# idiap/IdiapTTS

Measured on AMD Instinct MI355X. Metric: acoustic frames/sec (train), higher is better.
Workload: dtype f32

## Files before the change

### idiaptts_amd/csrc/sparse_wgrad.hip

```cpp
#include <algorithm>
#include <atomic>

#include "common.h"

namespace itts {

constexpr int kWgMaxK = 512;
constexpr int kTile = 256;
constexpr int kSlab = 64;
constexpr int kWgWaves = 16;
constexpr int kOwners = 64;
constexpr int kSlots = 8;
constexpr int kStrip = 32;
constexpr int kBlock = 16;
constexpr int kGroup = 4;
constexpr int kHeaderBytes = kSlots * 2;
constexpr int kFirstBytes = kBlock * 8;
constexpr int kOverBytes = (kTile / kBlock - 1) * kBlock * 8;
constexpr int kPlanInv = kStrip + kOwners * kSlots;
constexpr int kPlanInts = kPlanInv + kWgMaxK;
constexpr int kHeavyCode = 0x1000;
constexpr int kRowBytes = kSlab * 4;
constexpr int kBufBytes = (kTile + 1) * kRowBytes;
constexpr int kTPitch = 513;
// ... 40 lines not shown
  if (part == parts) {
    const int h = lane & 31;
    const int hc = h < kStrip - 1 ? plan[h] : -1;
    if (!(hc >= 0 && hc < K)) {
      for (int i = 0; i < 32; ++i) {
        const int64_t m = m0 + 2 * i + (lane >> 5);
        strip[m * kStrip + h] = (m < M && h == kStrip - 1) ? 0x3f800000u : 0u;
      }
    }
    for (int pair = threadIdx.x; pair < kOwners * kSlots; pair += 256) {
      const int c = plan[kStrip + pair];
      if (!(c >= 0 && c < K))
        reinterpret_cast<uint16_t*>(streams + ((int64_t)tile * kOwners + pair / kSlots) * kHeaderBytes)[pair % kSlots] = 0;
    }
    return;
  }
  const int k = part * 64 + lane;
  const bool valid = k < K;
  const int code = valid ? plan[kPlanInv + k] : -1;
  const bool light = code >= 0 && code < kOwners * kSlots;
  const bool heavy = code >= kHeavyCode && code < kHeavyCode + kStrip - 1;
  uint32_t bits[64];
#pragma unroll
  for (int r = 0; r < 64; ++r) bits[r] = (valid && m0 + r < M) ? x[(m0 + r) * ldx + k] : 0u;
  int cnt = 0;
#pragma unroll
  for (int r = 0; r < 64; ++r) cnt += (bits[r] & 0x7fffffffu) != 0u ? 1 : 0;
  cnts[wave][lane] = cnt;
  __syncthreads();
  if (heavy) {
    uint32_t* dst = strip + m0 * kStrip + (code - kHeavyCode);
#pragma unroll
    for (int r = 0; r < 64; ++r) dst[r * kStrip] = bits[r];
  }
  if (!light) return;
  int before = 0, total = 0;
#pragma unroll
  for (int w = 0; w < 4; ++w) {
    const int c = cnts[w][lane];
    before += w < wave ? c : 0;
    total += c;
  }
  const int owner = code / kSlots, slot = code % kSlots;
  const int64_t pair = ((int64_t)tile * kOwners + owner) * kSlots + slot;
  int j = before;
#pragma unroll
  for (int r = 0; r < 64; ++r)
    if ((bits[r] & 0x7fffffffu) != 0u)
      *entry_of(streams, tiles, pair, j++) = make_int2((wave * 64 + r) * kRowBytes, (int)bits[r]);
  if (wave == 0) {
    const int end = (total + kBlock - 1) / kBlock * kBlock;
    for (int e = total; e < end; ++e) *entry_of(streams, tiles, pair, e) = make_int2(kTile * kRowBytes, 0);
    reinterpret_cast<uint16_t*>(streams + ((int64_t)tile * kOwners + owner) * kHeaderBytes)[slot] = (uint16_t)total;
  }
}

typedef float floatx16 __attribute__((ext_vector_type(16)));

template <int J>
__device__ __forceinline__ void col_slot(const char* buf, int lane_off, int2 e, float4& acc) {
  const int off = __builtin_amdgcn_update_dpp(0, e.x, 0x150 + J, 0xf, 0xf, false);
  const float v = __int_as_float(__builtin_amdgcn_update_dpp(0, e.y, 0x150 + J, 0xf, 0xf, false));
  const float4 d = *reinterpret_cast<const float4*>(buf + off + lane_off);
  acc.x = fmaf(v, d.x, acc.x); acc.y = fmaf(v, d.y, acc.y);
  acc.z = fmaf(v, d.z, acc.z); acc.w = fmaf(v, d.w, acc.w);
}
template <int FIRST>
__device__ __forceinline__ void col_group(const char* buf, int lane_off, int2 e, float4& acc) {
  col_slot<FIRST>(buf, lane_off, e, acc);
  col_slot<FIRST + 1>(buf, lane_off, e, acc);
  col_slot<FIRST + 2>(buf, lane_off, e, acc);
  col_slot<FIRST + 3>(buf, lane_off, e, acc);
}

__global__ __launch_bounds__(kWgWaves * 64) void sparse_wgrad_kernel(
    const float* __restrict__ dz, int64_t lddz, const float* __restrict__ strip, const char* __restrict__ streams,
    const int* __restrict__ plan, float* __restrict__ slabs, int64_t slab_stride, int lddw,
    float* __restrict__ bias_part, int64_t bias_stride, int64_t M, int N, int K, int tiles, int per, int ranges) {
  extern __shared__ float4 smem4[];
  char* smem = reinterpret_cast<char*>(smem4);
  float* smemf = reinterpret_cast<float*>(smem4);
  const int tid = threadIdx.x, lane = tid & 63;
  const int wave = __builtin_amdgcn_readfirstlane(tid >> 6);
  const int i16 = lane & 15, owner = wave * 4 + (lane >> 4);
  const int n0 = (int)(blockIdx.x / ranges) * kSlab;
  const int range = (int)(blockIdx.x % ranges);
  const int t_begin = range * per, t_end = std::min(tiles, t_begin + per);

  if (tid < 128) smemf[((tid >> 6) * kBufBytes + kTile * kRowBytes) / 4 + lane] = 0.f;

  const int srow = tid >> 4, c4 = (tid & 15) * 4, n = n0 + c4;
  auto load_tile = [&](int t, float4 (&st)[4]) {
#pragma unroll
    for (int p = 0; p < 4; ++p) {
      const int64_t m = (int64_t)t * kTile + p * 64 + srow;
      float4 v = make_float4(0.f, 0.f, 0.f, 0.f);
      if (m < M) {
        const float* src = dz + m * lddz + n;
        if (n + 4 <= N) {
          v = *reinterpret_cast<const float4*>(src);
        } else {
          if (n < N) v.x = src[0];
          if (n + 1 < N) v.y = src[1];
          if (n + 2 < N) v.z = src[2];
        }
      }
// ... 134 lines not shown
  static int cus = 0;
  if (cus == 0) {
    int dev = 0, n = 0;
    if (hipGetDevice(&dev) != hipSuccess ||
        hipDeviceGetAttribute(&n, hipDeviceAttributeMultiprocessorCount, dev) != hipSuccess || n <= 0)
      n = 256;
    cus = n;
  }
  return cus;
}

static void wgrad_ranges(int64_t M, int N, int* per, int* ranges) {
  const int64_t tiles = (M + kTile - 1) / kTile;
  const int slabs = (N + kSlab - 1) / kSlab;
  const int64_t want = std::max<int64_t>(1, std::min<int64_t>(wgrad_compute_units() / slabs, tiles));
  *per = (int)((tiles + want - 1) / want);
  *ranges = (int)((tiles + *per - 1) / *per);
}

static bool wgrad_shape_ok(int K, int64_t lddw) { return K <= kWgMaxK && lddw <= kWgMaxK; }

}

using namespace itts;

extern "C" int itts_sparse_cols_plan_ints(void) { return kPlanInts; }

extern "C" int itts_sparse_cols_layout(int64_t M, int K, int64_t out[3]) {
  ITTS_REQUIRE(out != nullptr, "null pointer");
  ITTS_REQUIRE(M >= 0 && K > 0 && K <= kWgMaxK, "bad sizes (K <= 512)");
  const ColsLayout l = cols_layout(M);
  out[0] = l.strip_off; out[1] = l.streams_off; out[2] = l.bytes;
  return ITTS_OK;
}

extern "C" int itts_sparse_cols_build(const float* d_x, int64_t ldx, int64_t M, int K, const int* d_plan, void* d_cols,
                                      void* stream) {
  ITTS_REQUIRE(d_plan && d_cols && (M == 0 || d_x), "null pointer");
  ITTS_REQUIRE(M >= 0 && K > 0 && K <= kWgMaxK && ldx >= K, "bad sizes (K <= 512)");
  ITTS_REQUIRE(aligned16(d_cols), "the column block must be 16-byte aligned");
  if (M == 0) return ITTS_OK;
  const ColsLayout l = cols_layout(M);
  const int parts = (K + 63) / 64;
  ITTS_REQUIRE(l.tiles * (parts + 1) < ((int64_t)1 << 31), "too many rows");
  char* base = static_cast<char*>(d_cols);
  hipLaunchKernelGGL(sparse_cols_build_kernel, dim3((unsigned)(l.tiles * (parts + 1))), dim3(256), 0,
                     as_stream(stream), reinterpret_cast<const uint32_t*>(d_x), ldx, M, K, parts, (int)l.tiles, d_plan,
                     reinterpret_cast<uint32_t*>(base + l.strip_off), base + l.streams_off);
  ITTS_LAUNCH_CHECK();
  g_wgrad_path[0].fetch_add(1, std::memory_order_relaxed);
  return ITTS_OK;
}

extern "C" int64_t itts_linear_bwd_weight_sparse_workspace_bytes(int64_t M, int N, int K, int64_t lddw) {
  if (M < 0 || N <= 0 || K <= 0 || lddw < K) return 0;
  const int64_t dense = itts_linear_bwd_weight_workspace_bytes(M, N, (int)lddw);
  if (M == 0 || !wgrad_shape_ok(K, lddw)) return dense;
  int per, ranges;
  wgrad_ranges(M, N, &per, &ranges);
  return std::max<int64_t>(dense, (int64_t)ranges * ((int64_t)N * lddw + N) * 4);
}

extern "C" int itts_linear_bwd_weight_sparse(const float* d_dz, int64_t lddz, const void* d_cols, const int* d_plan,
                                             const float* d_x, int64_t ldx, float* d_dw, int64_t lddw, float* d_db,
                                             int64_t M, int N, int K, void* d_workspace, int accumulate,
                                             void* stream) {
  ITTS_REQUIRE(d_dw && d_workspace && (M == 0 || (d_dz && d_x)), "null pointer");
  ITTS_REQUIRE(M >= 0 && N > 0 && K > 0 && lddz >= N && ldx >= K && lddw >= K, "bad sizes");
  ITTS_REQUIRE(lddw == K || ldx >= lddw, "x must be as wide as dw's rows (its pad columns zero)");
  const bool sparse = M > 0 && d_cols && d_plan && wgrad_shape_ok(K, lddw) && lddz % 4 == 0 && aligned16(d_dz) &&
                      aligned16(d_cols);
  if (!sparse) {
    if (M > 0) g_wgrad_path[2].fetch_add(1, std::memory_order_relaxed);
    return itts_linear_bwd_weight(d_dz, lddz, d_x, ldx, d_dw, d_db, M, N, (int)lddw, d_workspace, accumulate, stream);
  }
  hipStream_t s = as_stream(stream);
  ITTS_HIP_CHECK(itts::allow_dynamic_lds((const void*)sparse_wgrad_kernel, kWgLdsBytes));
  const ColsLayout l = cols_layout(M);
  int per, ranges;
  wgrad_ranges(M, N, &per, &ranges);
  const int slabs_n = (N + kSlab - 1) / kSlab;
  ITTS_REQUIRE((int64_t)slabs_n * ranges < ((int64_t)1 << 31), "too many workgroups");
  const int64_t n = (int64_t)N * lddw;
  const bool merged = d_db && d_db == d_dw + n && N % 4 == 0 && n % 4 == 0;
  float* ws = static_cast<float*>(d_workspace);
  float* bias_part = !d_db ? nullptr : (merged ? ws + n : ws + (int64_t)ranges * n);
  const char* base = static_cast<const char*>(d_cols);
  hipLaunchKernelGGL(sparse_wgrad_kernel, dim3((unsigned)(slabs_n * ranges)), dim3(kWgWaves * 64), kWgLdsBytes, s, d_dz,
                     lddz, reinterpret_cast<const float*>(base + l.strip_off), base + l.streams_off, d_plan, ws,
                     merged ? n + N : n, (int)lddw, bias_part, merged ? n + N : (int64_t)N, M, N, K, (int)l.tiles, per,
                     ranges);
  ITTS_LAUNCH_CHECK();
  g_wgrad_path[1].fetch_add(1, std::memory_order_relaxed);
  if (merged) return reduce_slabs(ws, ranges, n + N, d_dw, accumulate, s);
  int rc = reduce_slabs(ws, ranges, n, d_dw, accumulate, s);
  if (rc || !d_db) return rc;
  return reduce_slabs(bias_part, ranges, (int64_t)N, d_db, accumulate, s);
}

extern "C" int itts_sparse_wgrad_counts(int64_t out[3]) {
  ITTS_REQUIRE(out != nullptr, "null pointer");
  for (int i = 0; i < 3; ++i) out[i] = g_wgrad_path[i].load(std::memory_order_relaxed);
  return ITTS_OK;
}
```

### idiaptts_amd/lib.py

```python
import ctypes
import os
from ctypes import POINTER, c_char_p, c_double, c_float, c_int, c_int64, c_uint8, c_void_p

_HERE = os.path.dirname(os.path.abspath(__file__))
LIB_PATH = os.path.join(_HERE, "_lib", "libidiaptts_amd.so")

_lib = None


class IttsError(RuntimeError):
    pass


_P = c_void_p

_SIGNATURES = {
    "itts_abi_version": (c_int, []),
    "itts_last_error": (c_char_p, []),
    "itts_device_count": (c_int, []),
    "itts_release_scratch": (c_int, []),
    "itts_defer_reductions": (c_int, [c_int]),
    "itts_reduce_deferred": (c_int, [_P]),
    "itts_scratch_pool_stats": (c_int, [POINTER(c_int64), POINTER(c_int64), POINTER(c_int64)]),
    "itts_comm_version": (c_int, []),
# ... 32 lines not shown
                                      POINTER(c_int64), c_int, c_int, _P, c_int64, _P]),
    "itts_feature_stats_workspace_bytes": (c_int64, [c_int, c_int]),
    "itts_feature_stats": (c_int, [_P, c_int64, c_int64, c_int, c_int, c_int, c_int, _P, _P, _P,
                                   _P]),
    "itts_linear_fwd": (c_int, [_P, c_int64, _P, _P, _P, c_int64, c_int64, c_int, c_int, c_int,
                                _P]),
    "itts_rows_gather_f32": (c_int, [_P, c_int64, c_int64, _P, c_int64, c_int, _P, _P, c_int64, c_int, _P]),
    "itts_mlpg_plan_create": (c_int, [_P, c_int, POINTER(c_void_p)]),
    "itts_mlpg_plan_destroy": (None, [_P]),
    "itts_mlpg_plan_frames": (c_int64, [_P]),
    "itts_mlpg_generation_planned": (c_int, [_P, _P, c_int, c_int64, c_int, c_int, _P, _P, c_int64, c_int, _P, _P]),
    "itts_mlpg_choose_form": (c_int, [c_int, c_int, c_int64, c_int64, c_int]),
    "itts_mlpg_set_override": (c_int, [c_int, c_int, c_int]),
    "itts_mlpg_get_override": (c_int, [POINTER(c_int), POINTER(c_int), POINTER(c_int)]),
    "itts_mlpg_last_form": (c_int, []),
    "itts_mlpg_adjoint_scratch_bytes": (c_int64, [c_int64, c_int]),
    "itts_mlpg_adjoint": (c_int, [_P, c_int, c_int64, c_int, c_int, _P, POINTER(c_int64), c_int, _P, c_int, c_int64,
                                  c_int, _P, _P]),
    "itts_mlpg_adjoint_planned": (c_int, [_P, _P, c_int, c_int64, c_int, c_int, _P, _P, c_int, c_int64, c_int, _P, _P]),
    "itts_mlpg_adjoint_choose_form": (c_int, [c_int, c_int, c_int64, c_int64]),
    "itts_mlpg_adjoint_set_override": (c_int, [c_int]),
    "itts_mlpg_adjoint_get_override": (c_int, []),
    "itts_mlpg_adjoint_last_form": (c_int, []),
    "itts_sqrt_inplace_f64": (c_int, [_P, c_int64, _P]),
    "itts_square_inplace_f64": (c_int, [_P, c_int64, _P]),
    "itts_stft": (c_int, [_P, POINTER(c_int64), POINTER(c_int64), POINTER(c_int64), c_int, c_int, c_int, c_int, _P,
                          c_int, _P, c_int64, _P]),
    "itts_stft_mel": (c_int, [_P, POINTER(c_int64), POINTER(c_int64), POINTER(c_int64), c_int, c_int, c_int, c_int,
                              _P, _P, _P, c_int, _P, c_int64, _P]),
    "itts_mel_project": (c_int, [_P, c_int64, c_int, c_int64, _P, _P, c_int, _P, c_int64, _P]),
    "itts_griffinlim": (c_int, [_P, _P, _P, _P, POINTER(c_int64), c_int, c_int, c_int, c_int, _P, c_int, c_double,
                                c_int, _P, _P]),
    "itts_griffinlim_tile_frames": (c_int, [c_int, c_int]),
    "itts_mel_inverse": (c_int, [_P, c_int64, c_int, c_int64, c_int, c_int, _P, _P, _P, _P, c_double, c_double, c_int,
                                 c_int, _P, c_int64, c_int, _P, _P]),
    "itts_batch_pad_gather_f32": (c_int, [_P, c_int64, c_int64, _P, _P, c_int, c_int64, c_int, c_int, _P, c_int64, _P,
                                          _P, c_int64, _P, _P]),
    "itts_batch_pack_rows_f32": (c_int, [_P, c_int64, _P, _P, c_int, c_int64, c_int, c_int, _P, c_int64, c_int,
                                         c_int64, c_int64, _P]),
    "itts_batch_concat_rows_f32": (c_int, [_P, c_int64, c_int64, _P, _P, _P, c_int, c_int64, c_int, _P, c_int64, c_int,
                                           _P]),
    "itts_batch_pad_colsum_workspace_bytes": (c_int64, [c_int64, c_int]),
    "itts_batch_pad_colsum_f32": (c_int, [_P, c_int64, _P, c_int, c_int64, c_int, c_int, _P, c_int, _P, _P]),
    "itts_linear_fwd_mse_workspace_bytes": (c_int64, [c_int64, c_int]),
    "itts_linear_fwd_mse": (c_int, [_P, c_int64, _P, _P, _P, c_int64, _P, c_double, c_float, c_int64,
                                    c_int, c_int, _P, _P, c_int64, _P, _P]),
    "itts_sparse_rows_layout": (c_int, [c_int64, c_int, POINTER(c_int64)]),
    "itts_sparse_rows_build": (c_int, [_P, c_int64, c_int64, c_int, _P, c_int, _P]),
    "itts_linear_fwd_sparse": (c_int, [_P, _P, c_int64, _P, _P, _P, c_int64, c_int64, c_int, c_int, c_int, _P]),
    "itts_sparse_path_counts": (c_int, [POINTER(c_int64)]),
    "itts_sparse_cols_plan_ints": (c_int, []),
    "itts_sparse_cols_layout": (c_int, [c_int64, c_int, POINTER(c_int64)]),
    "itts_sparse_cols_build": (c_int, [_P, c_int64, c_int64, c_int, _P, _P, _P]),
    "itts_linear_bwd_weight_sparse_workspace_bytes": (c_int64, [c_int64, c_int, c_int, c_int64]),
    "itts_linear_bwd_weight_sparse": (c_int, [_P, c_int64, _P, _P, _P, c_int64, _P, c_int64, _P, c_int64, c_int,
                                              c_int, _P, c_int, _P]),
    "itts_sparse_wgrad_counts": (c_int, [POINTER(c_int64)]),
    "itts_act_bwd": (c_int, [_P, _P, _P, c_int64, c_int, _P]),
    "itts_linear_bwd_input": (c_int, [_P, c_int64, _P, _P, c_int64, _P, c_int64, c_int, c_int64,
                                      c_int, c_int, _P]),
    "itts_linear_bwd_weight_workspace_bytes": (c_int64, [c_int64, c_int, c_int]),
    "itts_linear_bwd_weight": (c_int, [_P, c_int64, _P, c_int64, _P, _P, c_int64, c_int, c_int,
                                       _P, c_int, _P]),
    "itts_linear_bwd": (c_int, [_P, c_int64, _P, c_int64, _P, _P, _P, _P, c_int64, _P, c_int64, c_int,
                                c_int64, c_int, c_int, _P, c_int, _P]),
    "itts_conv1d_fwd": (c_int, [_P, c_int64, _P, _P, _P, c_int64, c_int, c_int, c_int, c_int, c_int,
                                c_int, c_int, c_int, c_int, _P]),
    "itts_conv1d_bwd_input": (c_int, [_P, c_int64, _P, _P, c_int64, _P, c_int64, c_int, c_int, c_int,
                                      c_int, c_int, c_int, c_int, c_int, c_int, _P]),
    "itts_conv1d_bwd_weight_workspace_bytes": (c_int64, [c_int, c_int, c_int, c_int, c_int, c_int,
                                                         c_int]),
    "itts_conv1d_bwd_weight": (c_int, [_P, c_int64, _P, c_int64, _P, _P, c_int, c_int, c_int, c_int,
                                       c_int, c_int, c_int, c_int, _P, c_int, _P]),
    "itts_conv1d_plan": (c_int, [c_int, c_int, c_int, c_int, c_int, c_int, c_int, c_int, c_int, POINTER(c_int),
                                 POINTER(c_int), POINTER(c_int64)]),
    "itts_layernorm_fwd": (c_int, [_P, c_int64, _P, _P, _P, c_int64, _P, _P, c_int64, c_int, c_double, c_int, _P]),
    "itts_layernorm_workspace_bytes": (c_int64, [c_int64, c_int]),
    "itts_layernorm_bwd": (c_int, [_P, c_int64, _P, c_int64, _P, c_int64, _P, _P, _P, _P, c_int64, _P, _P, c_int64,
                                   c_int, c_int, _P, _P]),
    "itts_allpass_warp_fwd": (c_int, [_P, c_int64, _P, _P, _P, _P, c_int64, c_int64, c_int, c_int, _P]),
    "itts_allpass_warp_bwd": (c_int, [_P, c_int64, _P, c_int64, _P, _P, _P, _P, c_int64, _P, c_int64, c_int, c_int,
                                      _P]),
    "itts_time_pool_plan": (c_int, [c_int, c_int64, c_int, POINTER(c_int), POINTER(c_int), POINTER(c_int64)]),
    "itts_time_pool_fwd": (c_int, [_P, c_int64, _P, c_int, c_int64, c_int, c_int, c_int, _P, c_int64, _P, _P]),
    "itts_time_pool_bwd": (c_int, [_P, c_int64, _P, c_int, c_int64, c_int, c_int, c_int, _P, c_int64, _P]),
    "itts_vae_reparam_fwd": (c_int, [_P, c_int64, _P, c_int64, _P, c_int64, c_int64, c_int, _P]),
    "itts_vae_reparam_bwd": (c_int, [_P, c_int64, _P, c_int64, _P, c_int64, _P, c_int64, _P, c_int64, _P, c_int64,
                                     c_int64, c_int, _P]),
    "itts_vae_kld_workspace_bytes": (c_int64, [c_int64, c_int]),
    "itts_vae_kld": (c_int, [_P, c_int64, _P, c_int64, _P, c_int64, c_int, _P, _P, c_int64, _P, c_int64, _P, _P, _P]),
    "itts_xent_plan": (c_int, [c_int64, c_int, c_int, POINTER(c_int), POINTER(c_int)]),
    "itts_softmax_xent_workspace_bytes": (c_int64, [c_int64, c_int]),
    "itts_softmax_xent": (c_int, [_P, c_int64, _P, _P, _P, c_int64, c_int, c_int64, _P, _P, _P, c_int64, _P, _P]),
    "itts_softmax_xent_strided_workspace_bytes": (c_int64, [c_int, c_int64]),
    "itts_softmax_xent_strided": (c_int, [_P, _P, _P, _P, c_int, c_int, c_int64, c_int, c_int64, _P, _P, _P, _P, _P]),
    "itts_class_counts": (c_int, [_P, c_int64, _P, c_int64, c_int, _P, _P, _P, _P]),
    "itts_masked_mse_workspace_bytes": (c_int64, [c_int64, c_int]),
    "itts_masked_mse": (c_int, [_P, c_int64, _P, c_int64, _P, c_int64, c_int, c_double, c_float,
                                _P, _P, c_int64, _P, _P]),
    "itts_weighted_loss": (c_int, [_P, c_int64, _P, c_int64, _P, c_int64, c_int, c_int, _P, _P,
                                   c_int64, _P, c_int64, _P, _P]),
    "itts_cheaptrick_mcep": (c_int, [_P, POINTER(c_int64), _P, POINTER(c_int64), c_int, c_int,
                                     c_double, c_int, c_double, _P, c_int, c_double, c_double,
                                     c_int, c_int, c_double, _P, c_int64, _P, _P, _P]),
    "itts_mcep": (c_int, [_P, c_int64, c_int, c_int, c_double, c_double, c_int, c_int, c_double,
                          _P, c_int64, _P, _P, _P]),
# ... 149 lines not shown
```

### idiaptts_amd/native_ff.py

```python
import math

import torch

from . import ops


def _pad4(n):
    return (n + 3) // 4 * 4


SPARSE_INPUT_MAX_DENSITY = 0.18

SPARSE_WGRAD_MAX_DENSITY = 0.09


class FlatFFModel:

    def __init__(self, dims=(425, 512, 512, 187), acts=("tanh", "tanh", None), device="cuda",
                 seed=0, state_dict=None, sparse_input=None, sparse_wgrad=None):
        assert len(acts) == len(dims) - 1
        self.dims = tuple(int(d) for d in dims)
        self.acts = [ops.act_code(a) for a in acts]
        self.device = torch.device(device)
        self.in_pitch = _pad4(self.dims[0])
        self.layout = []
        off = 0
        for li, (K, N) in enumerate(zip(self.dims[:-1], self.dims[1:])):
            kp = _pad4(K) if li == 0 else K
            w_off = off
            off += _pad4(N * kp)
            b_off = off
            off += _pad4(N)
            self.layout.append((w_off, b_off, N, K, kp))
        self.numel = off
        self.params = torch.zeros(off, dtype=torch.float32, device=self.device)
        self.grads = torch.zeros_like(self.params)
        self.exp_avg = torch.zeros_like(self.params)
        self.exp_avg_sq = torch.zeros_like(self.params)
        self.step_count = 0
        self._buffers = {}
        self.sparse_input = None if sparse_input is None else bool(sparse_input)
        self._lists = None
        self.sparse_wgrad = None if sparse_wgrad is None else bool(sparse_wgrad)
        self._col_plan = None
        self._cols = None
        if state_dict is None:
            state_dict = self.reference_init(self.dims, seed)
        self.load_layers(state_dict)

    @staticmethod
    def reference_init(dims, seed):
        g = torch.Generator().manual_seed(seed)
        layers = []
        for K, N in zip(dims[:-1], dims[1:]):
            bound = 1.0 / math.sqrt(K)
            w = (torch.rand(N, K, generator=g) * 2 - 1) * bound
            b = (torch.rand(N, generator=g) * 2 - 1) * bound
            layers.append((w, b))
        return layers

    @staticmethod
    def from_module(model, device=None):
        from .nn.modules import LinearAct
        inner = getattr(model, "model", model)
        layers, acts = [], []
        for group in getattr(inner, "layer_groups", []):
            seq = getattr(group, "module", None)
            if not isinstance(seq, torch.nn.Sequential):
                return None
# ... 73 lines not shown
    def _decide_sparse_input(self, x):
        self._lists = ops.sparse_rows_build(x, lists=self._lists, want_record=True)
        self.sparse_input = self._lists.density() <= SPARSE_INPUT_MAX_DENSITY

    def _use_sparse_wgrad(self, x):
        fits = self.dims[0] <= ops.SPARSE_COLS_MAX_K
        if self.sparse_wgrad is None:
            self.sparse_wgrad = False
            if self.sparse_input and fits:
                plan = ops.sparse_cols_plan(x, K=self.dims[0])
                if plan.density <= SPARSE_WGRAD_MAX_DENSITY:
                    self.sparse_wgrad, self._col_plan = True, plan
        if not self.sparse_wgrad:
            return False
        if self._col_plan is None and fits:
            self._col_plan = ops.sparse_cols_plan(x, K=self.dims[0])
        return True

    def loss_and_backward(self, x, target, row_valid, n_valid_global, reduce_group=None, reduce=False):
        self._pending = []
        x = self.pack_input(x)
        if self.sparse_input is None:
            self._decide_sparse_input(x)
        self._wgrad_sparse_now = self._use_sparse_wgrad(x)
        if reduce:
            return self._loss_and_backward(x, target, row_valid, n_valid_global, reduce_group, reduce)
        with ops.deferred_reductions():
            return self._loss_and_backward(x, target, row_valid, n_valid_global, reduce_group, False)

    def _loss_and_backward(self, x, target, row_valid, n_valid_global, reduce_group, reduce):
        M = x.shape[0]
        n = len(self.layout)
        if self.acts[-1] in (None, ops.ACT_NONE) and n > 1:
            hs = self.forward(x, n_layers=n - 1, sparse=bool(self.sparse_input))
            loss, dz = ops.linear_fwd_mse(hs[-1], self.weight_padded(n - 1), self.bias(n - 1), target,
                                          row_valid, n_valid_global,
                                          grad=self._rows_buffer("dz_out", M, self.dims[-1]))
            hs.append(None)
        else:
            hs = self.forward(x, sparse=bool(self.sparse_input))
            loss, dz = ops.masked_mse(hs[-1], target, row_valid, n_valid_global,
                                      grad=self._rows_buffer("dz_out", M, self.dims[-1]))
            if self.acts[-1] != ops.ACT_NONE:
                dz = ops.act_bwd(dz, hs[-1], self.acts[-1])
        for i in range(n - 1, -1, -1):
            inp = hs[i - 1] if i > 0 else x
            dz_in = None
            if i > 0:
                dz_in = self._rows_buffer("dz%d" % (i & 1), M, self.layout[i][3])
                ops.linear_bwd(dz, inp, self.weight_padded(i), self.weight_padded(i, self.grads),
                               self.bias(i, self.grads), dz_in, yprev=hs[i - 1], act_prev=self.acts[i - 1])
            elif self._wgrad_sparse_now:
                if self._col_plan is not None:
                    self._cols = ops.sparse_cols_build(x, self._col_plan, K=self.dims[0], cols=self._cols)
                ops.linear_bwd_weight_sparse(dz, x, self._cols if self._col_plan is not None else None,
                                             self._col_plan, dw=self.weight_padded(i, self.grads),
                                             db=self.bias(i, self.grads), K=self.dims[0])
            else:
                ops.linear_bwd_weight(dz, inp, dw=self.weight_padded(i, self.grads),
                                      db=self.bias(i, self.grads))
            if reduce:
                from .parallel import allreduce_flat_
                w_off, b_off, N, _, _ = self.layout[i]
                work = allreduce_flat_(self.grads[w_off:b_off + _pad4(N)], reduce_group, async_op=True)
                if work is not None:
                    self._pending.append(work)
            if i > 0:
                dz = dz_in
        return loss

    def train_step(self, x, target, row_valid, n_valid_global, lr=1e-3, betas=(0.9, 0.999),
                   eps=1e-8, weight_decay=0.0, process_group=None, world_size=1,
                   clip_norm_kind=None, clip_max_norm=0.0, clip_value=None, ema_shadow=None,
                   ema_decay=0.0):
        from . import parallel
        dist_on = world_size > 1 or parallel._active(process_group)
        loss = self.loss_and_backward(x, target, row_valid, n_valid_global, reduce_group=process_group,
                                      reduce=dist_on)
        for work in self._pending:
            work.wait()
        self._pending = []
        self.step_count += 1
        if clip_norm_kind is None and not clip_value and ema_shadow is None:
            ops.adam_step(self.params, self.grads, self.exp_avg, self.exp_avg_sq, self.step_count,
                          lr=lr, betas=betas, eps=eps, weight_decay=weight_decay)
            return loss
        accum = None
        if clip_norm_kind is not None:
            if getattr(self, "_norm_accum", None) is None:
                self._norm_accum = torch.zeros(1, dtype=torch.float32, device=self.device)
            accum = ops.grad_norm_accum(self.grads, self._norm_accum, clip_norm_kind)
        ops.adam_step_fused(self.params, self.grads, self.exp_avg, self.exp_avg_sq,
                            self.step_count, lr=lr, betas=betas, eps=eps,
                            weight_decay=weight_decay, norm_accum=accum,
                            norm_kind=clip_norm_kind if clip_norm_kind is not None else 2,
                            clip_max_norm=clip_max_norm, clip_value=clip_value or 0.0,
                            ema_shadow=ema_shadow, ema_decay=ema_decay)
        return loss


def flops_per_frame(dims, skip_first_dgrad=True):
    f = 0
    for i, (K, N) in enumerate(zip(dims[:-1], dims[1:])):
        f += 2 * N * K * (2 if (i == 0 and skip_first_dgrad) else 3)
    return f
```

### idiaptts_amd/ops.py

```python
import collections
import contextlib
import ctypes
import threading

import torch

from . import lib as _lib

ACT_NONE, ACT_TANH, ACT_RELU = 0, 1, 2
(ACT_SIGMOID, ACT_LOGSIGMOID, ACT_SOFTPLUS, ACT_SOFTSIGN, ACT_LEAKY_RELU, ACT_ELU, ACT_CELU, ACT_SELU, ACT_HARDTANH,
 ACT_RELU6, ACT_HARDSIGMOID) = range(3, 14)
ACT_TORCH_NAME = {ACT_TANH: "Tanh", ACT_RELU: "ReLU", ACT_SIGMOID: "Sigmoid", ACT_LOGSIGMOID: "LogSigmoid",
                  ACT_SOFTPLUS: "Softplus", ACT_SOFTSIGN: "Softsign", ACT_LEAKY_RELU: "LeakyReLU", ACT_ELU: "ELU",
                  ACT_CELU: "CELU", ACT_SELU: "SELU", ACT_HARDTANH: "Hardtanh", ACT_RELU6: "ReLU6",
                  ACT_HARDSIGMOID: "Hardsigmoid"}
ACT_BY_NAME = {None: ACT_NONE, "none": ACT_NONE, "linear": ACT_NONE}
ACT_BY_NAME.update({name.lower(): code for code, name in ACT_TORCH_NAME.items()})
CONV_ACTS = (ACT_NONE, ACT_TANH, ACT_RELU)


def act_code(act, allowed=None, where="Linear"):
    code = act if isinstance(act, int) else ACT_BY_NAME.get(act.lower() if isinstance(act, str) else act)
    if code is None or code not in (allowed if allowed is not None else range(ACT_HARDSIGMOID + 1)):
        raise NotImplementedError("{} activation {!r} is not implemented".format(where, act))
# ... 675 lines not shown

    def __init__(self, col_counts, rows, device, heavy_density=SPARSE_COLS_HEAVY_DENSITY):
        counts = [int(c) for c in col_counts]
        K = len(counts)
        if not 0 < K <= SPARSE_COLS_MAX_K:
            raise ValueError("a column plan holds 1 .. {} columns, got {}".format(SPARSE_COLS_MAX_K, K))
        order = sorted(range(K), key=lambda k: (-counts[k], k))
        self.heavy = [k for k in order if counts[k] > heavy_density * rows][:SPARSE_COLS_HEAVY]
        taken = set(self.heavy)
        self.owners = [[] for _ in range(SPARSE_COLS_OWNERS)]
        load = [0] * SPARSE_COLS_OWNERS
        for k in order:
            if k in taken:
                continue
            o = min((o for o in range(SPARSE_COLS_OWNERS) if len(self.owners[o]) < SPARSE_COLS_SLOTS),
                    key=lambda o: (load[o], len(self.owners[o]), o))
            self.owners[o].append(k)
            load[o] += counts[k]
        self.K = K
        self.density = sum(counts) / float(max(rows * K, 1))
        table = [-1] * int(_lib.load().itts_sparse_cols_plan_ints())
        inverse = SPARSE_COLS_HEAVY + 1 + SPARSE_COLS_OWNERS * SPARSE_COLS_SLOTS
        for h, k in enumerate(self.heavy):
            table[h] = k
            table[inverse + k] = 0x1000 + h
        for o, cols in enumerate(self.owners):
            for s, k in enumerate(cols):
                table[SPARSE_COLS_HEAVY + 1 + o * SPARSE_COLS_SLOTS + s] = k
                table[inverse + k] = o * SPARSE_COLS_SLOTS + s
        self.table = torch.tensor(table, dtype=torch.int32, device=device)


def sparse_cols_plan(x, K=None, heavy_density=SPARSE_COLS_HEAVY_DENSITY):
    K = x.shape[1] if K is None else int(K)
    counts = (x[:, :K] != 0).sum(dim=0).tolist()
    return SparseColsPlan(counts, x.shape[0], x.device, heavy_density)


class SparseCols(object):

    def __init__(self, M, K, device, block=None):
        out = (ctypes.c_int64 * 3)()
        _lib.check(_lib.load().itts_sparse_cols_layout(M, K, out), "itts_sparse_cols_layout")
        self.M, self.K = int(M), int(K)
        self._strip_off, self._streams_off, self.nbytes = (int(v) for v in out)
        if block is None or block.numel() < self.nbytes:
            block = torch.empty(max(self.nbytes, 16), dtype=torch.uint8, device=device)
        self.block = block

    def strip(self):
        return self.block[self._strip_off:self._streams_off].view(torch.float32).view(-1, 32)


def sparse_cols_build(x, plan, K=None, cols=None):
    _need(x, torch.float32, "x")
    ldx = _rows(x, "x")
    M = x.shape[0]
    K = x.shape[1] if K is None else int(K)
    if K > x.shape[1]:
        raise ValueError("K exceeds the width of x")
    if plan.K != K:
        raise ValueError("the plan was made for {} columns, not {}".format(plan.K, K))
    out = SparseCols(M, K, x.device, cols.block if cols is not None else None)
    _lib.check(_lib.load().itts_sparse_cols_build(_ptr(x), ldx, M, K, _ptr(plan.table), _ptr(out.block), _stream()),
               "itts_sparse_cols_build")
    return out


def linear_bwd_weight_sparse(dz, x, cols, plan, dw=None, db=None, accumulate=False, want_bias=True, K=None):
    L = _lib.load()
    _need(dz, torch.float32, "dz")
    _need(x, torch.float32, "x")
    M, N = dz.shape
    K = (cols.K if cols is not None else x.shape[1]) if K is None else int(K)
    if cols is not None and (cols.M != M or cols.K != K or plan is None or plan.K != K):
        raise ValueError("the column data were built for another shape or without this plan")
    if dw is None:
        dw = torch.empty((N, K), dtype=torch.float32, device=dz.device)
    if dw.dim() != 2 or dw.shape[0] != N or dw.shape[1] < K or not dw.is_contiguous():
        raise ValueError("dw must be contiguous [N, >= K]")
    if db is None and want_bias:
        db = torch.empty((N,), dtype=torch.float32, device=dz.device)
    lddw = dw.shape[1]
    ws = _workspace(L.itts_linear_bwd_weight_sparse_workspace_bytes(M, N, K, lddw), dz.device)
    _lib.check(L.itts_linear_bwd_weight_sparse(_ptr(dz), _rows(dz, "dz"),
                                               _ptr(cols.block) if cols is not None else None,
                                               _ptr(plan.table) if plan is not None else None, _ptr(x), _rows(x, "x"),
                                               _ptr(dw), lddw, _ptr(db), M, N, K, _ptr(ws), 1 if accumulate else 0,
                                               _stream()), "itts_linear_bwd_weight_sparse")
    return dw, db


SparseWgradCounts = collections.namedtuple("SparseWgradCounts", "col_builds dw_sparse dw_dense")


def sparse_wgrad_counts():
    out = (ctypes.c_int64 * 3)()
    _lib.check(_lib.load().itts_sparse_wgrad_counts(out), "itts_sparse_wgrad_counts")
    return SparseWgradCounts(*[int(v) for v in out])


def conv1d_out_len(T_in, kernel_size, padding, dilation):
    return T_in + 2 * padding - dilation * (kernel_size - 1)


def _conv_rows(t, name):
    if t.dim() != 3:
        raise ValueError("{} must be 3-D [B, T, C] (batch_first) or [T, B, C]".format(name))
    C = t.shape[2]
    ld = t.stride(1) if t.shape[1] > 1 else (t.stride(0) if t.shape[0] > 1 else C)
    ok = (t.stride(2) == 1 or C == 1) and ld >= C and (t.shape[0] == 1 or t.stride(0) == t.shape[1] * ld)
    if ok and ld != C and ld % 4 == 0:
        ok = t.storage_offset() + t.shape[0] * t.shape[1] * ld <= t.untyped_storage().nbytes() // 4
    if ok:
        return t, ld
    return t.clone(memory_format=torch.contiguous_format), C
# ... 1349 lines not shown
```

### include/idiaptts_amd.h

```cpp
#ifndef IDIAPTTS_AMD_H
#define IDIAPTTS_AMD_H

#include <stdint.h>

#ifdef __cplusplus
extern "C" {
#endif

#define ITTS_OK 0
#define ITTS_E_INVALID (-1)
#define ITTS_E_HIP (-2)
#define ITTS_E_UNSUPPORTED (-3)

int itts_abi_version(void);
const char* itts_last_error(void);
int itts_device_count(void);
int itts_scratch_pool_stats(int64_t* reserved, int64_t* used, int64_t* keep_threshold);

int itts_release_scratch(void);

int itts_defer_reductions(int on);
int itts_reduce_deferred(void* stream);

#define ITTS_F32 0
// ... 131 lines not shown
                               float* d_dst, int64_t ld_dst, int dst_width, void* stream);
int64_t itts_batch_pad_colsum_workspace_bytes(int64_t n_rows, int width);
int itts_batch_pad_colsum_f32(const float* d_x, int64_t ld_x, const int64_t* d_lens, int n_utts, int64_t t_max,
                              int width, int batch_first, float* d_out, int out_width, void* d_workspace,
                              void* stream);

#define ITTS_ACT_NONE 0
#define ITTS_ACT_TANH 1
#define ITTS_ACT_RELU 2
#define ITTS_ACT_SIGMOID 3
#define ITTS_ACT_LOGSIGMOID 4
#define ITTS_ACT_SOFTPLUS 5
#define ITTS_ACT_SOFTSIGN 6
#define ITTS_ACT_LEAKY_RELU 7
#define ITTS_ACT_ELU 8
#define ITTS_ACT_CELU 9
#define ITTS_ACT_SELU 10
#define ITTS_ACT_HARDTANH 11
#define ITTS_ACT_RELU6 12
#define ITTS_ACT_HARDSIGMOID 13
int itts_linear_fwd(const float* d_x, int64_t ldx, const float* d_w, const float* d_b,
                    float* d_y, int64_t ldy, int64_t M, int N, int K, int act, void* stream);
int64_t itts_linear_fwd_mse_workspace_bytes(int64_t M, int N);
int itts_linear_fwd_mse(const float* d_x, int64_t ldx, const float* d_w, const float* d_b,
                        const float* d_target, int64_t ldt, const uint8_t* d_row_valid, double n_valid,
                        float loss_weight, int64_t M, int N, int K, float* d_loss, float* d_dz,
                        int64_t lddz, void* d_workspace, void* stream);

int itts_act_bwd(const float* d_dy, const float* d_y, float* d_dz, int64_t n_elem, int act,
                 void* stream);
int itts_linear_bwd_input(const float* d_dz, int64_t lddz, const float* d_w, float* d_dx,
                          int64_t lddx, const float* d_yprev, int64_t ldyp, int act_prev,
                          int64_t M, int N, int K, void* stream);
int64_t itts_linear_bwd_weight_workspace_bytes(int64_t M, int N, int K);
int itts_linear_bwd_weight(const float* d_dz, int64_t lddz, const float* d_x, int64_t ldx,
                           float* d_dw, float* d_db, int64_t M, int N, int K,
                           void* d_workspace, int accumulate, void* stream);
int itts_linear_bwd(const float* d_dz, int64_t lddz, const float* d_x, int64_t ldx, const float* d_w,
                    float* d_dw, float* d_db, float* d_dx, int64_t lddx, const float* d_yprev,
                    int64_t ldyp, int act_prev, int64_t M, int N, int K, void* d_workspace,
                    int accumulate, void* stream);

int itts_sparse_rows_layout(int64_t M, int K, int64_t out[4]);
int itts_sparse_rows_build(const float* d_x, int64_t ldx, int64_t M, int K, void* d_lists, int want_record,
                           void* stream);
int itts_linear_fwd_sparse(const void* d_lists, const float* d_x, int64_t ldx, const float* d_w, const float* d_b,
                           float* d_y, int64_t ldy, int64_t M, int N, int K, int act, void* stream);
int itts_sparse_path_counts(int64_t out[3]);

int itts_sparse_cols_plan_ints(void);
int itts_sparse_cols_layout(int64_t M, int K, int64_t out[3]);
int itts_sparse_cols_build(const float* d_x, int64_t ldx, int64_t M, int K, const int* d_plan, void* d_cols,
                           void* stream);
int64_t itts_linear_bwd_weight_sparse_workspace_bytes(int64_t M, int N, int K, int64_t lddw);
int itts_linear_bwd_weight_sparse(const float* d_dz, int64_t lddz, const void* d_cols, const int* d_plan,
                                  const float* d_x, int64_t ldx, float* d_dw, int64_t lddw, float* d_db, int64_t M,
                                  int N, int K, void* d_workspace, int accumulate, void* stream);
int itts_sparse_wgrad_counts(int64_t out[3]);

int itts_conv1d_fwd(const float* d_x, int64_t ldx, const float* d_w, const float* d_b, float* d_y,
                    int64_t ldy, int B, int T_in, int Cin, int Cout, int Kw, int pad, int dil,
                    int batch_first, int act, void* stream);
int itts_conv1d_bwd_input(const float* d_dz, int64_t lddz, const float* d_w, float* d_dx, int64_t lddx,
                          const float* d_yprev, int64_t ldyp, int act_prev, int B, int T_in, int Cin,
                          int Cout, int Kw, int pad, int dil, int batch_first, void* stream);
int64_t itts_conv1d_bwd_weight_workspace_bytes(int B, int T_in, int Cin, int Cout, int Kw, int pad, int dil);
int itts_conv1d_bwd_weight(const float* d_dz, int64_t lddz, const float* d_x, int64_t ldx, float* d_dw,
                           float* d_db, int B, int T_in, int Cin, int Cout, int Kw, int pad, int dil,
                           int batch_first, void* d_workspace, int accumulate, void* stream);
int itts_conv1d_plan(int product, int B, int T_in, int Cin, int Cout, int Kw, int pad, int dil, int vec,
                     int* tile_cols, int* slabs, int64_t* kchunk);

int itts_layernorm_fwd(const float* d_x, int64_t ldx, const float* d_gamma, const float* d_beta,
                       float* d_y, int64_t ldy, float* d_mean, float* d_rstd, int64_t N, int D,
                       double eps, int act, void* stream);
int64_t itts_layernorm_workspace_bytes(int64_t N, int D);
int itts_layernorm_bwd(const float* d_dy, int64_t lddy, const float* d_x, int64_t ldx,
                       const float* d_y, int64_t ldy, const float* d_mean, const float* d_rstd,
                       const float* d_gamma, float* d_dx, int64_t lddx, float* d_dgamma,
                       float* d_dbeta, int64_t N, int D, int act, void* d_workspace, void* stream);

int itts_allpass_warp_fwd(const float* d_x, int64_t ldx, const float* d_alpha, const float* d_mean,
                          const float* d_std_dev, float* d_y, int64_t ldy, int64_t M, int D, int N,
                          void* stream);
int itts_allpass_warp_bwd(const float* d_dy, int64_t lddy, const float* d_x, int64_t ldx,
                          const float* d_alpha, const float* d_mean, const float* d_std_dev, float* d_dx,
                          int64_t lddx, float* d_dalpha, int64_t M, int D, int N, void* stream);

#define ITTS_POOL_LAST 0
#define ITTS_POOL_MEAN 1
int itts_time_pool_plan(int n_utts, int64_t t_max, int width, int* segments, int* split, int64_t* workspace_bytes);
int itts_time_pool_fwd(const float* d_x, int64_t ldx, const int64_t* d_lens, int n_utts, int64_t t_max, int width,
                       int batch_first, int mode, float* d_y, int64_t ldy, void* d_workspace, void* stream);
int itts_time_pool_bwd(const float* d_dy, int64_t lddy, const int64_t* d_lens, int n_utts, int64_t t_max, int width,
                       int batch_first, int mode, float* d_dx, int64_t lddx, void* stream);
int itts_vae_reparam_fwd(const float* d_h, int64_t ldh, const float* d_eps, int64_t lde, float* d_z, int64_t ldz,
                         int64_t M, int L, void* stream);
int itts_vae_reparam_bwd(const float* d_dz, int64_t lddz, const float* d_dmu, int64_t lddmu, const float* d_dlv,
                         int64_t lddlv, const float* d_h, int64_t ldh, const float* d_eps, int64_t lde, float* d_dh,
                         int64_t lddh, int64_t M, int L, void* stream);
int64_t itts_vae_kld_workspace_bytes(int64_t M, int L);
int itts_vae_kld(const float* d_mu, int64_t ldmu, const float* d_lv, int64_t ldlv, const float* d_w, int64_t M, int L,
                 float* d_loss, float* d_dmu, int64_t lddmu, float* d_dlv, int64_t lddlv, float* d_elem,
                 void* d_workspace, void* stream);

#define ITTS_XENT_ROWS 0
// ... 199 lines not shown
```

Before: 41.33 million.

## Build sparse weight-grad column lists from existing row lists instead of dense input

Adds a kernel that builds the per-tile column entry streams for the sparse weight-gradient path from the already-built sparse row lists, rather than rescanning the dense input matrix. Each workgroup handles a 256-row tile, marks row membership per list with LDS bitmask atomics, prefix-sums across waves, then scatters entries, heavy-column strip values and padding. The aim is to avoid reading the full dense x in the backward pass when forward row lists exist. It uses a large LDS footprint per block and more complex scatter logic.

After: 42.21 million (median of 6 runs). 1.02x the previous value.

```diff
diff --git a/idiaptts_amd/csrc/sparse_wgrad.hip b/idiaptts_amd/csrc/sparse_wgrad.hip
--- a/idiaptts_amd/csrc/sparse_wgrad.hip
+++ b/idiaptts_amd/csrc/sparse_wgrad.hip
@@ -116,6 +116,159 @@
     const int end = (total + kBlock - 1) / kBlock * kBlock;
     for (int e = total; e < end; ++e) *entry_of(streams, tiles, pair, e) = make_int2(kTile * kRowBytes, 0);
     reinterpret_cast<uint16_t*>(streams + ((int64_t)tile * kOwners + owner) * kHeaderBytes)[slot] = (uint16_t)total;
+  }
+}
+
+constexpr int kFromRowsWaves = 16;
+constexpr int kFromRowsPairs = kTile / kFromRowsWaves / 2;
+constexpr int kLists = kOwners * kSlots;
+constexpr int kFromRowsLdsBytes = kLists * kFirstBytes + kTile * kStrip * 4 + kFromRowsWaves * kLists * 4 + kWgMaxK * 4;
+
+__global__ __launch_bounds__(kFromRowsWaves * 64) void sparse_cols_from_rows_kernel(
+    const int* __restrict__ counts, const int4* __restrict__ entries2, int64_t pitch2, int64_t M, int K, int tiles,
+    const int* __restrict__ plan, uint32_t* __restrict__ strip, char* __restrict__ streams) {
+  constexpr int T = kFromRowsWaves * 64;
+  extern __shared__ uint4 from_rows_lds[];
+  int2* first = reinterpret_cast<int2*>(from_rows_lds);
+  uint32_t* tile_strip = reinterpret_cast<uint32_t*>(first + kLists * kBlock);
+  uint32_t* words = tile_strip + kTile * kStrip;
+  int* inverse = reinterpret_cast<int*>(words + kFromRowsWaves * kLists);
+  const int tid = threadIdx.x, lane = tid & 63, l32 = lane & 31;
+  const int wave = __builtin_amdgcn_readfirstlane(tid >> 6);
+  const int tile = (int)blockIdx.x;
+  const int64_t m0 = (int64_t)tile * kTile;
+  const int row0 = wave * 2 * kFromRowsPairs + (lane >> 5);
+
+  int code_of_tid = -1;
+  if (tid < K) {
+    const int code = plan[kPlanInv + tid];
+    if ((code >= 0 && code < kLists) || (code >= kHeavyCode && code < kHeavyCode + kStrip - 1)) code_of_tid = code;
+  }
+  int cnt[kFromRowsPairs];
+  int4 head[kFromRowsPairs];
+#pragma unroll
+  for (int q = 0; q < kFromRowsPairs; ++q) {
+    const int64_t m = m0 + row0 + 2 * q;
+    const bool in = m < M && l32 < pitch2;
+    cnt[q] = in ? std::min(counts[m], (int)(2 * pitch2)) : 0;
+    head[q] = in ? entries2[m * pitch2 + l32] : make_int4(-1, 0, -1, 0);
+  }
+
+  {
+    const uint4 neutral = make_uint4((uint32_t)(kTile * kRowBytes), 0u, (uint32_t)(kTile * kRowBytes), 0u);
+    uint4* first4 = reinterpret_cast<uint4*>(first);
+    for (int i = tid; i < kLists * kFirstBytes / 16; i += T) first4[i] = neutral;
+    uint4* strip4 = reinterpret_cast<uint4*>(tile_strip);
+    for (int i = tid; i < kTile * kStrip / 4; i += T) {
+      const bool ones = (i & 7) == 7 && m0 + (i >> 3) < M;
+      strip4[i] = make_uint4(0u, 0u, 0u, ones ? 0x3f800000u : 0u);
+    }
+    uint4* words4 = reinterpret_cast<uint4*>(words);
+    for (int i = tid; i < kFromRowsWaves * kLists / 4; i += T) words4[i] = make_uint4(0u, 0u, 0u, 0u);
+    if (tid < kWgMaxK) inverse[tid] = code_of_tid;
+  }
+  int most = 0;
+#pragma unroll
+  for (int q = 0; q < kFromRowsPairs; ++q) {
+    if (2 * l32 >= cnt[q]) head[q].x = -1;
+    if (2 * l32 + 1 >= cnt[q]) head[q].z = -1;
+    most = std::max(most, cnt[q]);
+  }
+  const bool further = std::max(most, __shfl_xor(most, 32, 64)) > 64;
+  __syncthreads();
+
+  uint32_t* my_words = words + wave * kLists;
+  auto code_of = [&](int k) { return (unsigned)k < (unsigned)K ? inverse[k] : -1; };
+  auto again = [&](int q, int j0) {
+    int4 e = j0 + 2 * l32 < cnt[q] ? entries2[(m0 + row0 + 2 * q) * pitch2 + j0 / 2 + l32] : make_int4(-1, 0, -1, 0);
+    if (j0 + 2 * l32 + 1 >= cnt[q]) e.z = -1;
+    e.x = code_of(e.x);
+    e.z = code_of(e.z);
+    return e;
+  };
+  auto mark = [&](int q, int code) {
+    if (code >= 0 && code < kLists) atomicOr(&my_words[code], 1u << (2 * q + (lane >> 5)));
+  };
+  auto place = [&](int q, int code, int value) {
+    const int row = 2 * q + (lane >> 5);
+    if (code >= 0 && code < kLists) {
+      const uint32_t word = my_words[code];
+      const int pos = (int)(word >> 16) + __popc(word & ((1u << row) - 1u));
+      const int2 out = make_int2((row0 + 2 * q) * kRowBytes, value);
+      if (pos < kBlock) first[code * kBlock + pos] = out;
+      else if (pos < kTile) *entry_of(streams, tiles, (int64_t)tile * kLists + code, pos) = out;
+    } else if (code >= kHeavyCode) {
+      tile_strip[(row0 + 2 * q) * kStrip + (code - kHeavyCode)] = (uint32_t)value;
+    }
+  };
+
+#pragma unroll
+  for (int q = 0; q < kFromRowsPairs; ++q) {
+    head[q].x = code_of(head[q].x);
+    head[q].z = code_of(head[q].z);
+  }
+#pragma unroll
+  for (int q = 0; q < kFromRowsPairs; ++q) {
+    mark(q, head[q].x);
+    mark(q, head[q].z);
+  }
+  if (further) {
+#pragma unroll
+    for (int q = 0; q < kFromRowsPairs; ++q)
+      for (int j0 = 64; j0 < cnt[q]; j0 += 64) {
+        const int4 e = again(q, j0);
+        mark(q, e.x);
+        mark(q, e.z);
+      }
+  }
+  __syncthreads();
+
+  if (tid < kLists) {
+    int run = 0;
+#pragma unroll
+    for (int w = 0; w < kFromRowsWaves; ++w) {
+      const uint32_t rows_of_wave = words[w * kLists + tid];
+      words[w * kLists + tid] = rows_of_wave | ((uint32_t)run << 16);
+      run += __popc(rows_of_wave);
+    }
+    reinterpret_cast<uint16_t*>(streams)[(int64_t)tile * kLists + tid] = (uint16_t)run;
+  }
+  __syncthreads();
+
+#pragma unroll
+  for (int q = 0; q < kFromRowsPairs; ++q) {
+    place(q, head[q].x, head[q].y);
+    place(q, head[q].z, head[q].w);
+  }
+  if (further) {
+#pragma unroll
+    for (int q = 0; q < kFromRowsPairs; ++q)
+      for (int j0 = 64; j0 < cnt[q]; j0 += 64) {
+        const int4 e = again(q, j0);
+        place(q, e.x, e.y);
+        place(q, e.z, e.w);
+      }
+  }
+  __syncthreads();
+
+  {
+    const uint4* first4 = reinterpret_cast<const uint4*>(first);
+    uint4* dst = reinterpret_cast<uint4*>(const_cast<char*>(firsts_of(streams, tiles)) +
+                                          (int64_t)tile * kLists * kFirstBytes);
+    for (int i = tid; i < kLists * kFirstBytes / 16; i += T) dst[i] = first4[i];
+    const uint4* strip4 = reinterpret_cast<const uint4*>(tile_strip);
+    uint4* sdst = reinterpret_cast<uint4*>(strip + m0 * kStrip);
+    for (int i = tid; i < kTile * kStrip / 4; i += T) sdst[i] = strip4[i];
+  }
+  {
+    const int list = tid & (kLists - 1);
+    const uint32_t last = words[(kFromRowsWaves - 1) * kLists + list];
+    const int total = (int)(last >> 16) + __popc(last & 0xffffu);
+    if (total > kBlock) {
+      const int end = (total + kBlock - 1) / kBlock * kBlock;
+      for (int e = total + (tid >> 9); e < end; e += T / kLists)
+        *entry_of(streams, tiles, (int64_t)tile * kLists + list, e) = make_int2(kTile * kRowBytes, 0);
+    }
   }
 }
 
@@ -356,6 +509,29 @@
   return ITTS_OK;
 }
 
+extern "C" int itts_sparse_cols_build_from_rows(const void* d_lists, int64_t M, int K_lists, int K, const int* d_plan,
+                                                void* d_cols, void* stream) {
+  ITTS_REQUIRE(d_plan && d_cols && (M == 0 || d_lists), "null pointer");
+  ITTS_REQUIRE(M >= 0 && K > 0 && K <= kWgMaxK && K_lists >= K && K_lists <= 65535,
+               "bad sizes (K <= 512, K <= K_lists <= 65535)");
+  ITTS_REQUIRE(aligned16(d_cols) && aligned16(d_lists), "the column and list blocks must be 16-byte aligned");
+  if (M == 0) return ITTS_OK;
+  int64_t rows[4];
+  if (int rc = itts_sparse_rows_layout(M, K_lists, rows)) return rc;
+  const ColsLayout l = cols_layout(M);
+  ITTS_REQUIRE(l.tiles < ((int64_t)1 << 31), "too many rows");
+  ITTS_HIP_CHECK(itts::allow_dynamic_lds((const void*)sparse_cols_from_rows_kernel, kFromRowsLdsBytes));
+  const char* lists = static_cast<const char*>(d_lists);
+  char* base = static_cast<char*>(d_cols);
+  hipLaunchKernelGGL(sparse_cols_from_rows_kernel, dim3((unsigned)l.tiles), dim3(kFromRowsWaves * 64),
+                     kFromRowsLdsBytes, as_stream(stream), reinterpret_cast<const int*>(lists + rows[0]),
+                     reinterpret_cast<const int4*>(lists + rows[1]), rows[2] / 2, M, K, (int)l.tiles, d_plan,
+                     reinterpret_cast<uint32_t*>(base + l.strip_off), base + l.streams_off);
+  ITTS_LAUNCH_CHECK();
+  g_wgrad_path[0].fetch_add(1, std::memory_order_relaxed);
+  return ITTS_OK;
+}
+
 extern "C" int64_t itts_linear_bwd_weight_sparse_workspace_bytes(int64_t M, int N, int K, int64_t lddw) {
   if (M < 0 || N <= 0 || K <= 0 || lddw < K) return 0;
   const int64_t dense = itts_linear_bwd_weight_workspace_bytes(M, N, (int)lddw);
diff --git a/idiaptts_amd/lib.py b/idiaptts_amd/lib.py
--- a/idiaptts_amd/lib.py
+++ b/idiaptts_amd/lib.py
@@ -108,6 +108,7 @@
     "itts_sparse_cols_plan_ints": (c_int, []),
     "itts_sparse_cols_layout": (c_int, [c_int64, c_int, POINTER(c_int64)]),
     "itts_sparse_cols_build": (c_int, [_P, c_int64, c_int64, c_int, _P, _P, _P]),
+    "itts_sparse_cols_build_from_rows": (c_int, [_P, c_int64, c_int, c_int, _P, _P, _P]),
     "itts_linear_bwd_weight_sparse_workspace_bytes": (c_int64, [c_int64, c_int, c_int, c_int64]),
     "itts_linear_bwd_weight_sparse": (c_int, [_P, c_int64, _P, _P, _P, c_int64, _P, c_int64, _P, c_int64, c_int,
                                               c_int, _P, c_int, _P]),
diff --git a/idiaptts_amd/native_ff.py b/idiaptts_amd/native_ff.py
--- a/idiaptts_amd/native_ff.py
+++ b/idiaptts_amd/native_ff.py
@@ -15,6 +15,8 @@
 
 
 class FlatFFModel:
+
+    cols_from_lists = True
 
     def __init__(self, dims=(425, 512, 512, 187), acts=("tanh", "tanh", None), device="cuda",
                  seed=0, state_dict=None, sparse_input=None, sparse_wgrad=None):
@@ -194,7 +196,9 @@
                                self.bias(i, self.grads), dz_in, yprev=hs[i - 1], act_prev=self.acts[i - 1])
             elif self._wgrad_sparse_now:
                 if self._col_plan is not None:
-                    self._cols = ops.sparse_cols_build(x, self._col_plan, K=self.dims[0], cols=self._cols)
+                    lists = self._lists if self.cols_from_lists and self.sparse_input else None
+                    self._cols = ops.sparse_cols_build(x, self._col_plan, K=self.dims[0], cols=self._cols,
+                                                       lists=lists)
                 ops.linear_bwd_weight_sparse(dz, x, self._cols if self._col_plan is not None else None,
                                              self._col_plan, dw=self.weight_padded(i, self.grads),
                                              db=self.bias(i, self.grads), K=self.dims[0])
diff --git a/idiaptts_amd/ops.py b/idiaptts_amd/ops.py
--- a/idiaptts_amd/ops.py
+++ b/idiaptts_amd/ops.py
@@ -751,7 +751,7 @@
         return self.block[self._strip_off:self._streams_off].view(torch.float32).view(-1, 32)
 
 
-def sparse_cols_build(x, plan, K=None, cols=None):
+def sparse_cols_build(x, plan, K=None, cols=None, lists=None):
     _need(x, torch.float32, "x")
     ldx = _rows(x, "x")
     M = x.shape[0]
@@ -761,6 +761,13 @@
     if plan.K != K:
         raise ValueError("the plan was made for {} columns, not {}".format(plan.K, K))
     out = SparseCols(M, K, x.device, cols.block if cols is not None else None)
+    if lists is not None:
+        if lists.M != M or lists.K < K:
+            raise ValueError("the row lists were built for another shape")
+        _lib.check(_lib.load().itts_sparse_cols_build_from_rows(_ptr(lists.block), M, lists.K, K, _ptr(plan.table),
+                                                                _ptr(out.block), _stream()),
+                   "itts_sparse_cols_build_from_rows")
+        return out
     _lib.check(_lib.load().itts_sparse_cols_build(_ptr(x), ldx, M, K, _ptr(plan.table), _ptr(out.block), _stream()),
                "itts_sparse_cols_build")
     return out
diff --git a/include/idiaptts_amd.h b/include/idiaptts_amd.h
--- a/include/idiaptts_amd.h
+++ b/include/idiaptts_amd.h
@@ -207,6 +207,8 @@
 int itts_sparse_cols_layout(int64_t M, int K, int64_t out[3]);
 int itts_sparse_cols_build(const float* d_x, int64_t ldx, int64_t M, int K, const int* d_plan, void* d_cols,
                            void* stream);
+int itts_sparse_cols_build_from_rows(const void* d_lists, int64_t M, int K_lists, int K, const int* d_plan,
+                                     void* d_cols, void* stream);
 int64_t itts_linear_bwd_weight_sparse_workspace_bytes(int64_t M, int N, int K, int64_t lddw);
 int itts_linear_bwd_weight_sparse(const float* d_dz, int64_t lddz, const void* d_cols, const int* d_plan,
                                   const float* d_x, int64_t ldx, float* d_dw, int64_t lddw, float* d_db, int64_t M,
```
